# lucidrains/vit-pytorch

Hardware: NVIDIA H100
Metric: images/sec ViT-B/16 224^2 bf16 fwd (higher is better)
Workload: dtype bf16

## Files before the change

vit_pytorch_b200/csrc/attention.cu:

```cuda
#include "common.cuh"
#include "host_util.h"

namespace b200 {

constexpr int ATT_QROWS = 128;
constexpr int ATT_THREADS = 256;

struct AttnParams {
  __nv_bfloat16* out;
  int N;
  const int32_t* cu_seqlens;
  const int32_t* tile_prefix;
  int num_seqs;
  int H, I;
  float scale_log2e;
};

template <int DH, int KB>
struct AttnSmem {
  static constexpr int N64 = DH / 64;
  static constexpr int N16 = (DH % 64) / 16;
  static_assert(N64 * 64 + N16 * 16 == DH, "dim_head must be a multiple of 16");
  static constexpr int Q64 = ATT_QROWS * 128;
  static constexpr int Q16 = ATT_QROWS * 32;
  static constexpr int KV64 = KB * 128;
  static constexpr int KV16 = KB * 32;
  static constexpr int K16_OFF = 2 * N64 * KV64;
  static constexpr int V16_OFF = K16_OFF + N16 * KV16;
  static constexpr int STAGE = 2 * (N64 * KV64 + N16 * KV16);
  static constexpr int STAGE_OFF = N64 * Q64 + N16 * Q16;
  static constexpr int BAR_OFF = STAGE_OFF + 2 * STAGE;
  static constexpr int BYTES = BAR_OFF + 5 * 8 + 1024;
};

constexpr int att_min_blocks(int dh, int kb) { return (dh == 64 && kb == 64) || dh == 32 ? 2 : 1; }

template <int DH, int KB, bool VARLEN, bool EMUL, bool MASK_SELF>
__global__ void __launch_bounds__(ATT_THREADS, att_min_blocks(DH, KB))
attention_kernel(const __grid_constant__ CUtensorMap tmQ, const __grid_constant__ CUtensorMap tmKV,
                 const __grid_constant__ CUtensorMap tmQ16, const __grid_constant__ CUtensorMap tmKV16,
                 const AttnParams p) {
  using L = AttnSmem<DH, KB>;
  constexpr int N64 = L::N64, N16 = L::N16;
  constexpr int NS = KB / 2;
  extern __shared__ uint8_t smem_raw[];
  uint8_t* smem = reinterpret_cast<uint8_t*>((reinterpret_cast<uintptr_t>(smem_raw) + 1023) & ~uintptr_t(1023));
  uint64_t* full = reinterpret_cast<uint64_t*>(smem + L::BAR_OFF);
  uint64_t* empty = full + 2;
  uint64_t* qbar = full + 4;

  const int h = blockIdx.y;
  int seq_start, len, q0;
  if (VARLEN) {
    const int tile = blockIdx.x;
    int lo = 0, hi = p.num_seqs - 1;
    while (lo < hi) {
      const int mid = (lo + hi + 1) >> 1;
      if (p.tile_prefix[mid] <= tile) lo = mid;
      else hi = mid - 1;
    }
    seq_start = p.cu_seqlens[lo];
    len = p.cu_seqlens[lo + 1] - seq_start;
    q0 = (tile - p.tile_prefix[lo]) * ATT_QROWS;
  } else {
    seq_start = blockIdx.z * p.N;
    len = p.N;
    q0 = blockIdx.x * ATT_QROWS;
  }
  const int nblocks = (len + KB - 1) / KB;
  const int colq = h * DH, colk = p.I + h * DH, colv = 2 * p.I + h * DH;
  const int tid = threadIdx.x;
  const int wg = tid >> 7, t = tid & 127, warp = t >> 5, lane = t & 31;

  auto issue_kv = [&](int blk) {
    const int st = blk & 1;
    uint8_t* sb = smem + L::STAGE_OFF + st * L::STAGE;
    const int row = seq_start + blk * KB;
    mbar_arrive_expect_tx(&full[st], L::STAGE);
#pragma unroll
    for (int c = 0; c < N64; ++c) {
      tma_load_2d(sb + c * L::KV64, &tmKV, &full[st], colk + 64 * c, row);
      tma_load_2d(sb + (N64 + c) * L::KV64, &tmKV, &full[st], colv + 64 * c, row);
    }
#pragma unroll
    for (int c = 0; c < N16; ++c) {
      tma_load_2d(sb + L::K16_OFF + c * L::KV16, &tmKV16, &full[st], colk + 64 * N64 + 16 * c, row);
      tma_load_2d(sb + L::V16_OFF + c * L::KV16, &tmKV16, &full[st], colv + 64 * N64 + 16 * c, row);
    }
  };

  if (tid == 0) {
    tma_prefetch_desc(&tmQ);
    tma_prefetch_desc(&tmKV);
    for (int i = 0; i < 2; ++i) {
      mbar_init(&full[i], 1);
      mbar_init(&empty[i], 2);
    }
    mbar_init(qbar, 1);
    fence_mbar_init();
  }
  __syncthreads();
  if (tid == 0) {
    mbar_arrive_expect_tx(qbar, L::STAGE_OFF);
#pragma unroll
    for (int c = 0; c < N64; ++c) tma_load_2d(smem + c * L::Q64, &tmQ, qbar, colq + 64 * c, seq_start + q0);
#pragma unroll
    for (int c = 0; c < N16; ++c)
      tma_load_2d(smem + N64 * L::Q64 + c * L::Q16, &tmQ16, qbar, colq + 64 * N64 + 16 * c, seq_start + q0);
    issue_kv(0);
    if (nblocks > 1) issue_kv(1);
  }

  float o[N64 > 0 ? N64 : 1][32], o16[N16 > 0 ? N16 : 1][8];
#pragma unroll
  for (int c = 0; c < N64; ++c)
#pragma unroll
    for (int i = 0; i < 32; ++i) o[c][i] = 0.f;
#pragma unroll
  for (int c = 0; c < N16; ++c)
#pragma unroll
    for (int i = 0; i < 8; ++i) o16[c][i] = 0.f;
  float m[2] = {-INFINITY, -INFINITY}, l[2] = {0.f, 0.f};
  const uint32_t qa = smem_u32(smem) + wg * 64 * 128;
  const uint32_t qa16 = smem_u32(smem + N64 * L::Q64) + wg * 64 * 32;
  const bool mask_self = MASK_SELF && len > 1;
  mbar_wait(qbar, 0);

  for (int kb = 0; kb < nblocks; ++kb) {
    const int st = kb & 1;
    const uint32_t ph = (kb >> 1) & 1;
    mbar_wait(&full[st], ph);
    const uint32_t sb = smem_u32(smem + L::STAGE_OFF + st * L::STAGE);

    float s[NS];
    wgmma_fence();
#pragma unroll
    for (int c = 0; c < N64; ++c)
#pragma unroll
      for (int k = 0; k < 4; ++k) {
        const uint64_t ad = make_wgmma_desc(qa + c * L::Q64, 1024, WGMMA_SW128) + 2 * k;
        const uint64_t bd = make_wgmma_desc(sb + c * L::KV64, 1024, WGMMA_SW128) + 2 * k;
        if constexpr (KB == 128) wgmma_m64n128k16(s, ad, bd, c != 0 || k != 0);
        else wgmma_m64n64k16(s, ad, bd, c != 0 || k != 0);
      }
#pragma unroll
    for (int c = 0; c < N16; ++c) {
      const uint64_t ad = make_wgmma_desc(qa16 + c * L::Q16, 256, WGMMA_SW32);
      const uint64_t bd = make_wgmma_desc(sb + L::K16_OFF + c * L::KV16, 256, WGMMA_SW32);
      if constexpr (KB == 128) wgmma_m64n128k16(s, ad, bd, N64 != 0 || c != 0);
      else wgmma_m64n64k16(s, ad, bd, N64 != 0 || c != 0);
    }
    wgmma_commit();
    wgmma_wait<0>();
    fence_regs(s);

    const int key0 = kb * KB + 2 * (lane & 3);
    float mx[2] = {m[0], m[1]};
#pragma unroll
    for (int j = 0; j < KB / 8; ++j)
#pragma unroll
      for (int e = 0; e < 4; ++e) {
        const int key = key0 + j * 8 + (e & 1);
        bool valid = key < len;
        if constexpr (MASK_SELF)
          valid = valid && !(mask_self && key == q0 + wg * 64 + warp * 16 + (lane >> 2) + 8 * (e >> 1));
        s[4 * j + e] = valid ? s[4 * j + e] * p.scale_log2e : -INFINITY;
        mx[e >> 1] = fmaxf(mx[e >> 1], s[4 * j + e]);
      }
#pragma unroll
    for (int r = 0; r < 2; ++r) {
      mx[r] = fmaxf(mx[r], __shfl_xor_sync(0xffffffffu, mx[r], 1));
      mx[r] = fmaxf(mx[r], __shfl_xor_sync(0xffffffffu, mx[r], 2));
      const float corr = fast_ex2(m[r] - mx[r]);
      l[r] *= corr;
#pragma unroll
      for (int c = 0; c < N64; ++c)
#pragma unroll
        for (int i = 0; i < 8; ++i) {
          o[c][4 * i + 2 * r] *= corr;
          o[c][4 * i + 2 * r + 1] *= corr;
        }
#pragma unroll
      for (int c = 0; c < N16; ++c)
#pragma unroll
        for (int i = 0; i < 2; ++i) {
          o16[c][4 * i + 2 * r] *= corr;
          o16[c][4 * i + 2 * r + 1] *= corr;
        }
      m[r] = mx[r];
    }
#pragma unroll
    for (int j = 0; j < KB / 8; ++j) {
#pragma unroll
      for (int r = 0; r < 2; ++r) {
        float e0, e1;
        const float x0 = s[4 * j + 2 * r] - m[r], x1 = s[4 * j + 2 * r + 1] - m[r];
        if (EMUL && (j & 1)) {
          exp2_emul2(f2_make(x0, x1), e0, e1);
          e0 = s[4 * j + 2 * r] == -INFINITY ? 0.f : e0;
          e1 = s[4 * j + 2 * r + 1] == -INFINITY ? 0.f : e1;
        } else {
          e0 = fast_ex2(x0);
          e1 = fast_ex2(x1);
        }
        s[4 * j + 2 * r] = e0;
        s[4 * j + 2 * r + 1] = e1;
        l[r] += e0 + e1;
      }
    }

    wgmma_fence();
#pragma unroll
    for (int kk = 0; kk < KB / 16; ++kk) {
      const uint32_t a[4] = {pack_bf16x2(s[8 * kk], s[8 * kk + 1]), pack_bf16x2(s[8 * kk + 2], s[8 * kk + 3]),
                             pack_bf16x2(s[8 * kk + 4], s[8 * kk + 5]), pack_bf16x2(s[8 * kk + 6], s[8 * kk + 7])};
#pragma unroll
      for (int c = 0; c < N64; ++c)
        wgmma_m64n64k16_rs_tb(o[c], a,
                              make_wgmma_desc_lbo(sb + (N64 + c) * L::KV64 + kk * 2048, 1024, 1024, WGMMA_SW128));
#pragma unroll
      for (int c = 0; c < N16; ++c)
        wgmma_m64n16k16_rs_tb(o16[c], a,
                              make_wgmma_desc_lbo(sb + L::V16_OFF + c * L::KV16 + kk * 512, 256, 256, WGMMA_SW32));
    }
    wgmma_commit();
    wgmma_wait<0>();
#pragma unroll
    for (int c = 0; c < N64; ++c) fence_regs(o[c]);
#pragma unroll
    for (int c = 0; c < N16; ++c) fence_regs(o16[c]);
    if (t == 0) mbar_arrive(&empty[st]);
    if (tid == 0 && kb + 2 < nblocks) {
      mbar_wait(&empty[st], ph);
      issue_kv(kb + 2);
    }
  }

#pragma unroll
  for (int r = 0; r < 2; ++r) {
    l[r] += __shfl_xor_sync(0xffffffffu, l[r], 1);
    l[r] += __shfl_xor_sync(0xffffffffu, l[r], 2);
    l[r] = 1.0f / l[r];
  }
  const int qr = q0 + wg * 64 + warp * 16 + (lane >> 2);
#pragma unroll
  for (int r = 0; r < 2; ++r) {
    const int row = qr + 8 * r;
    if (row >= len) continue;
    __nv_bfloat16* op = p.out + (long long)(seq_start + row) * p.I + h * DH + 2 * (lane & 3);
#pragma unroll
    for (int c = 0; c < N64; ++c)
#pragma unroll
      for (int j = 0; j < 8; ++j)
        *reinterpret_cast<uint32_t*>(op + 64 * c + j * 8) =
            pack_bf16x2(o[c][4 * j + 2 * r] * l[r], o[c][4 * j + 2 * r + 1] * l[r]);
#pragma unroll
    for (int c = 0; c < N16; ++c)
#pragma unroll
      for (int j = 0; j < 2; ++j)
        *reinterpret_cast<uint32_t*>(op + 64 * N64 + 16 * c + j * 8) =
            pack_bf16x2(o16[c][4 * j + 2 * r] * l[r], o16[c][4 * j + 2 * r + 1] * l[r]);
  }
}

template <int DH, int KB, bool VARLEN, bool EMUL, bool MASK_SELF>
static int launch_attention_t(const void* qkv, int T, const AttnParams& p, dim3 grid, cudaStream_t stream) {
  using L = AttnSmem<DH, KB>;
  CUtensorMap tm[4];
  const uint64_t dims[2] = {(uint64_t)3 * p.I, (uint64_t)T};
  const uint64_t strides[1] = {(uint64_t)3 * p.I * 2};
  const uint32_t qbox[2] = {64, ATT_QROWS}, kvbox[2] = {64, KB}, qbox16[2] = {16, ATT_QROWS}, kvbox16[2] = {16, KB};
  int rc = 0;
  if (L::N64) rc = encode_tmap_bf16(&tm[0], qkv, 2, dims, strides, qbox);
  if (!rc && L::N64) rc = encode_tmap_bf16(&tm[1], qkv, 2, dims, strides, kvbox);
  if (!rc && L::N16) rc = encode_tmap_bf16_sw(&tm[2], qkv, 2, dims, strides, qbox16, 32);
  if (!rc && L::N16) rc = encode_tmap_bf16_sw(&tm[3], qkv, 2, dims, strides, kvbox16, 32);
  if (rc) return rc;
  if (!L::N16) tm[2] = tm[0], tm[3] = tm[1];
  if (!L::N64) tm[0] = tm[2], tm[1] = tm[3];
  auto kern = attention_kernel<DH, KB, VARLEN, EMUL, MASK_SELF>;
  B200_ENSURE_SMEM(kern, L::BYTES);
  kern<<<grid, ATT_THREADS, L::BYTES, stream>>>(tm[0], tm[1], tm[2], tm[3], p);
  B200_CHECK_CUDA(cudaGetLastError());
  count_launch();
  return 0;
}

template <int DH, bool VARLEN>
static int launch_attention_dh(const void* qkv, int T, const AttnParams& p, int kb, bool emul, bool mask_self,
                               dim3 grid, cudaStream_t st) {
  if (mask_self) return launch_attention_t<DH, 64, VARLEN, false, true>(qkv, T, p, grid, st);
  if (kb == 128) return emul ? launch_attention_t<DH, 128, VARLEN, true, false>(qkv, T, p, grid, st)
                             : launch_attention_t<DH, 128, VARLEN, false, false>(qkv, T, p, grid, st);
  return emul ? launch_attention_t<DH, 64, VARLEN, true, false>(qkv, T, p, grid, st)
              : launch_attention_t<DH, 64, VARLEN, false, false>(qkv, T, p, grid, st);
}

template <bool VARLEN>
static int launch_attention(const void* qkv, int T, const AttnParams& p, int dh, int kb, bool emul, bool mask_self,
                            dim3 grid, cudaStream_t st) {
  switch (dh) {
    case 32: return launch_attention_dh<32, VARLEN>(qkv, T, p, kb, emul, mask_self, grid, st);
    case 80: return launch_attention_dh<80, VARLEN>(qkv, T, p, kb, emul, mask_self, grid, st);
    case 128: return launch_attention_dh<128, VARLEN>(qkv, T, p, kb, emul, mask_self, grid, st);
    default: return launch_attention_dh<64, VARLEN>(qkv, T, p, kb, emul, mask_self, grid, st);
  }
}

static std::atomic<int> g_attn_mode{0};
static std::atomic<int> g_attn_emul{0};
static std::atomic<int> g_varlen_mode{0};

}

using namespace b200;

extern "C" int b200vit_debug_set(int key, int value) {
  switch (key) {
    case 1: g_attn_mode = value; return 0;
    case 11: g_varlen_mode = value; return 0;
    case 12: gemm_set_block_n(value); return 0;
    case 13: g_attn_emul = value; return 0;
    case 14: gemm_set_direct_store(value); return 0;
    default: return B200VIT_ERR_INVALID;
  }
}

extern "C" int b200vit_attention(const void* qkv, void* out, int B, int N, int H, int dh, float scale, void* stream) {
  return b200vit_attention_ex(qkv, out, B, N, H, dh, scale, 0, stream);
}

extern "C" int b200vit_attention_ex(const void* qkv, void* out, int B, int N, int H, int dh, float scale, int flags,
                                    void* stream) {
  B200_CHECK_ARG(qkv && out, "attention: null pointer");
  B200_CHECK_ARG(B > 0 && N > 0 && H > 0, "attention: bad shape B=%d N=%d H=%d", B, N, H);
  B200_CHECK_ARG(head_width_ok(dh), "attention: dim_head=%d not supported by this build (32, 64, 80 or 128)", dh);
  B200_CHECK_ARG(N <= 512, "attention: N=%d > 512 goes through b200vit_attention_varlen", N);
  B200_CHECK_ARG((reinterpret_cast<uintptr_t>(qkv) & 15) == 0 && (reinterpret_cast<uintptr_t>(out) & 15) == 0,
                 "attention: pointers must be 16-byte aligned");
  B200_CHECK_ARG(B <= 65535, "attention: B=%d exceeds the grid", B);
  B200_CHECK_ARG((flags & ~B200VIT_ATTN_MASK_SELF) == 0, "attention: unknown flags 0x%x", flags);
  AttnParams p{};
  p.out = reinterpret_cast<__nv_bfloat16*>(out);
  p.N = N;
  p.H = H;
  p.I = H * dh;
  p.scale_log2e = scale * 1.4426950408889634f;
  const dim3 grid((N + ATT_QROWS - 1) / ATT_QROWS, H, B);
  return launch_attention<false>(qkv, B * N, p, dh, g_attn_mode.load() == 2 ? 128 : 64, g_attn_emul.load() != 0,
                                 (flags & B200VIT_ATTN_MASK_SELF) != 0, grid, reinterpret_cast<cudaStream_t>(stream));
}

extern "C" int b200vit_attention_varlen(const void* qkv, void* out, const int32_t* cu_seqlens_dev,
                                        const int32_t* tile_prefix_dev, int num_seqs, int total_tokens, int total_tiles,
                                        int H, int dh, float scale, void* stream) {
  return b200vit_attention_varlen_ex(qkv, out, cu_seqlens_dev, tile_prefix_dev, num_seqs, total_tokens, total_tiles, H,
                                     dh, scale, 0, stream);
}

extern "C" int b200vit_attention_varlen_ex(const void* qkv, void* out, const int32_t* cu_seqlens_dev,
                                           const int32_t* tile_prefix_dev, int num_seqs, int total_tokens,
                                           int total_tiles, int H, int dh, float scale, int flags, void* stream) {
  B200_CHECK_ARG(qkv && out && cu_seqlens_dev && tile_prefix_dev, "attention_varlen: null pointer");
  B200_CHECK_ARG(num_seqs > 0 && total_tokens > 0 && total_tiles > 0 && H > 0, "attention_varlen: bad shape");
  B200_CHECK_ARG(head_width_ok(dh), "attention_varlen: dim_head=%d not supported by this build (32, 64, 80 or 128)",
                 dh);
  B200_CHECK_ARG((reinterpret_cast<uintptr_t>(qkv) & 15) == 0 && (reinterpret_cast<uintptr_t>(out) & 15) == 0,
                 "attention_varlen: pointers must be 16-byte aligned");
  B200_CHECK_ARG(H <= 65535, "attention_varlen: H=%d exceeds the grid", H);
  B200_CHECK_ARG((flags & ~B200VIT_ATTN_MASK_SELF) == 0, "attention_varlen: unknown flags 0x%x", flags);
  AttnParams p{};
  p.out = reinterpret_cast<__nv_bfloat16*>(out);
  p.cu_seqlens = cu_seqlens_dev;
  p.tile_prefix = tile_prefix_dev;
  p.num_seqs = num_seqs;
  p.H = H;
  p.I = H * dh;
  p.scale_log2e = scale * 1.4426950408889634f;
  const int mode = g_varlen_mode.load();
  const dim3 grid(total_tiles, H, 1);
  return launch_attention<true>(qkv, total_tokens, p, dh, mode == 1 ? 128 : 64, mode == 2,
                                (flags & B200VIT_ATTN_MASK_SELF) != 0, grid, reinterpret_cast<cudaStream_t>(stream));
}
```

vit_pytorch_b200/csrc/common.cuh:

```cuda
#pragma once
#include <cuda.h>
#include <cuda_runtime.h>
#include <cuda_bf16.h>
#include <stdint.h>

namespace b200 {

__device__ __forceinline__ uint32_t smem_u32(const void* p) {
  return static_cast<uint32_t>(__cvta_generic_to_shared(p));
}
__device__ __forceinline__ uint64_t globaltimer_ns() {
  uint64_t t;
  asm volatile("mov.u64 %0, %%globaltimer;" : "=l"(t));
  return t;
}
__device__ __forceinline__ bool elect_one() {
  uint32_t pred;
  asm volatile(
      "{\n\t.reg .pred p;\n\t"
      "elect.sync _|p, 0xffffffff;\n\t"
      "selp.u32 %0, 1, 0, p;\n\t}"
      : "=r"(pred));
  return pred != 0;
}

__device__ __forceinline__ void pdl_wait() { asm volatile("griddepcontrol.wait;" ::: "memory"); }
__device__ __forceinline__ void pdl_launch_dependents() { asm volatile("griddepcontrol.launch_dependents;" ::: "memory"); }

template <int N>
__device__ __forceinline__ void setmaxnreg_inc() { asm volatile("setmaxnreg.inc.sync.aligned.u32 %0;" ::"n"(N)); }
template <int N>
__device__ __forceinline__ void setmaxnreg_dec() { asm volatile("setmaxnreg.dec.sync.aligned.u32 %0;" ::"n"(N)); }

__device__ __forceinline__ void mbar_init(uint64_t* bar, uint32_t count) {
  asm volatile("mbarrier.init.shared::cta.b64 [%0], %1;" ::"r"(smem_u32(bar)), "r"(count) : "memory");
}
__device__ __forceinline__ void fence_mbar_init() {
  asm volatile("fence.mbarrier_init.release.cluster;" ::: "memory");
}
__device__ __forceinline__ void sts_v4(uint32_t addr, uint32_t x, uint32_t y, uint32_t z, uint32_t w) {
  asm volatile("st.shared.v4.b32 [%0], {%1, %2, %3, %4};" ::"r"(addr), "r"(x), "r"(y), "r"(z), "r"(w) : "memory");
}
__device__ __forceinline__ void sts_v4f(uint32_t addr, float x, float y, float z, float w) {
  asm volatile("st.shared.v4.f32 [%0], {%1, %2, %3, %4};" ::"r"(addr), "f"(x), "f"(y), "f"(z), "f"(w) : "memory");
}
__device__ __forceinline__ float4 lds_v4f(uint32_t addr) {
  float4 r;
  asm volatile("ld.shared.v4.f32 {%0, %1, %2, %3}, [%4];" : "=f"(r.x), "=f"(r.y), "=f"(r.z), "=f"(r.w) : "r"(addr) : "memory");
  return r;
}
__device__ __forceinline__ void fence_proxy_async_smem() {
  asm volatile("fence.proxy.async.shared::cta;" ::: "memory");
}
__device__ __forceinline__ void mbar_arrive_expect_tx(uint64_t* bar, uint32_t bytes) {
  asm volatile("mbarrier.arrive.expect_tx.shared::cta.b64 _, [%0], %1;" ::"r"(smem_u32(bar)), "r"(bytes) : "memory");
}
__device__ __forceinline__ void mbar_arrive(uint64_t* bar) {
  asm volatile("mbarrier.arrive.shared::cta.b64 _, [%0];" ::"r"(smem_u32(bar)) : "memory");
}
__device__ __forceinline__ uint32_t mbar_try_wait(uint64_t* bar, uint32_t parity) {
  uint32_t ok;
  asm volatile(
      "{\n\t.reg .pred p;\n\t"
      "mbarrier.try_wait.parity.shared::cta.b64 p, [%1], %2;\n\t"
      "selp.u32 %0, 1, 0, p;\n\t}"
      : "=r"(ok)
      : "r"(smem_u32(bar)), "r"(parity)
      : "memory");
  return ok;
}
#ifndef B200VIT_WATCHDOG_NS
#define B200VIT_WATCHDOG_NS 4000000000ull
#endif
__device__ __forceinline__ void mbar_wait(uint64_t* bar, uint32_t parity) {
  if (mbar_try_wait(bar, parity)) return;
  uint64_t t0 = globaltimer_ns();
  uint32_t spins = 0;
  while (!mbar_try_wait(bar, parity)) {
    if (((++spins) & 0x3FFu) == 0) {
      if (globaltimer_ns() - t0 > B200VIT_WATCHDOG_NS) __trap();
    }
  }
}

__device__ __forceinline__ void tma_prefetch_desc(const CUtensorMap* tm) {
  asm volatile("prefetch.tensormap [%0];" ::"l"(reinterpret_cast<uint64_t>(tm)) : "memory");
}
__device__ __forceinline__ void tma_prefetch_l2_2d(const CUtensorMap* tm, int c0, int c1) {
  asm volatile("cp.async.bulk.prefetch.tensor.2d.L2.global.tile [%0, {%1, %2}];" ::"l"(reinterpret_cast<uint64_t>(tm)),
               "r"(c0), "r"(c1)
               : "memory");
}
__device__ __forceinline__ void tma_load_2d(void* smem_dst, const CUtensorMap* tm, uint64_t* bar, int c0, int c1) {
  asm volatile(
      "cp.async.bulk.tensor.2d.shared::cluster.global.mbarrier::complete_tx::bytes [%0], [%1, {%3, %4}], [%2];"
      ::"r"(smem_u32(smem_dst)), "l"(reinterpret_cast<uint64_t>(tm)), "r"(smem_u32(bar)), "r"(c0), "r"(c1)
      : "memory");
}
__device__ __forceinline__ void tma_load_3d(void* smem_dst, const CUtensorMap* tm, uint64_t* bar, int c0, int c1,
                                            int c2) {
  asm volatile(
      "cp.async.bulk.tensor.3d.shared::cluster.global.mbarrier::complete_tx::bytes [%0], [%1, {%3, %4, %5}], [%2];"
      ::"r"(smem_u32(smem_dst)), "l"(reinterpret_cast<uint64_t>(tm)), "r"(smem_u32(bar)), "r"(c0), "r"(c1), "r"(c2)
      : "memory");
}
__device__ __forceinline__ void tma_load_4d(void* smem_dst, const CUtensorMap* tm, uint64_t* bar, int c0, int c1,
                                            int c2, int c3) {
  asm volatile(
      "cp.async.bulk.tensor.4d.shared::cluster.global.mbarrier::complete_tx::bytes [%0], [%1, {%3, %4, %5, %6}], [%2];"
      ::"r"(smem_u32(smem_dst)), "l"(reinterpret_cast<uint64_t>(tm)), "r"(smem_u32(bar)), "r"(c0), "r"(c1), "r"(c2),
      "r"(c3)
      : "memory");
}
__device__ __forceinline__ void tma_load_5d(void* smem_dst, const CUtensorMap* tm, uint64_t* bar, int c0, int c1,
                                            int c2, int c3, int c4) {
  asm volatile(
      "cp.async.bulk.tensor.5d.shared::cluster.global.mbarrier::complete_tx::bytes [%0], [%1, {%3, %4, %5, %6, %7}], "
      "[%2];"
      ::"r"(smem_u32(smem_dst)), "l"(reinterpret_cast<uint64_t>(tm)), "r"(smem_u32(bar)), "r"(c0), "r"(c1), "r"(c2),
      "r"(c3), "r"(c4)
      : "memory");
}
__device__ __forceinline__ void tma_store_2d(const CUtensorMap* tm, const void* smem_src, int c0, int c1) {
  asm volatile("cp.async.bulk.tensor.2d.global.shared::cta.bulk_group [%0, {%2, %3}], [%1];" ::"l"(
                   reinterpret_cast<uint64_t>(tm)),
               "r"(smem_u32(smem_src)), "r"(c0), "r"(c1)
               : "memory");
}
__device__ __forceinline__ void tma_store_commit() { asm volatile("cp.async.bulk.commit_group;" ::: "memory"); }
template <int N>
__device__ __forceinline__ void tma_store_wait_read() {
  asm volatile("cp.async.bulk.wait_group.read %0;" ::"n"(N) : "memory");
}
template <int N>
__device__ __forceinline__ void tma_store_wait() {
  asm volatile("cp.async.bulk.wait_group %0;" ::"n"(N) : "memory");
}

__device__ __forceinline__ uint64_t make_wgmma_desc(uint32_t smem_addr, uint32_t sbo_bytes, uint32_t swizzle) {
  uint64_t d = 0;
  d |= static_cast<uint64_t>((smem_addr & 0x3FFFFu) >> 4);
  d |= static_cast<uint64_t>(1u) << 16;
  d |= static_cast<uint64_t>((sbo_bytes >> 4) & 0x3FFFu) << 32;
  d |= static_cast<uint64_t>(swizzle) << 62;
  return d;
}
__device__ __forceinline__ uint64_t make_wgmma_desc_lbo(uint32_t smem_addr, uint32_t lbo_bytes, uint32_t sbo_bytes,
                                                        uint32_t swizzle) {
  return (make_wgmma_desc(smem_addr, sbo_bytes, swizzle) & ~(0x3FFFull << 16)) |
         (static_cast<uint64_t>((lbo_bytes >> 4) & 0x3FFFu) << 16);
}
constexpr uint32_t WGMMA_SW128 = 1;
constexpr uint32_t WGMMA_SW32 = 3;

__device__ __forceinline__ void wgmma_fence() { asm volatile("wgmma.fence.sync.aligned;" ::: "memory"); }
__device__ __forceinline__ void wgmma_commit() { asm volatile("wgmma.commit_group.sync.aligned;" ::: "memory"); }
template <int N>
__device__ __forceinline__ void wgmma_wait() { asm volatile("wgmma.wait_group.sync.aligned %0;" ::"n"(N) : "memory"); }
template <int R>
__device__ __forceinline__ void fence_regs(float (&d)[R]) {
#pragma unroll
  for (int i = 0; i < R; ++i) asm volatile("" : "+f"(d[i])::"memory");
}

__device__ __forceinline__ void wgmma_m64n128k16(float (&d)[64], uint64_t a_desc, uint64_t b_desc, uint32_t scale_d) {
  asm volatile(
      "{\n\t.reg .pred p;\n\t"
      "setp.ne.b32 p, %66, 0;\n\t"
      "wgmma.mma_async.sync.aligned.m64n128k16.f32.bf16.bf16 "
      "{"
      "%0, %1, %2, %3, %4, %5, %6, %7, %8, %9, %10, %11, %12, %13, %14, %15, "
      "%16, %17, %18, %19, %20, %21, %22, %23, %24, %25, %26, %27, %28, %29, %30, %31, "
      "%32, %33, %34, %35, %36, %37, %38, %39, %40, %41, %42, %43, %44, %45, %46, %47, "
      "%48, %49, %50, %51, %52, %53, %54, %55, %56, %57, %58, %59, %60, %61, %62, %63"
      "}, %64, %65, p, 1, 1, 0, 0;\n\t}"
      : "+f"(d[0]), "+f"(d[1]), "+f"(d[2]), "+f"(d[3]), "+f"(d[4]), "+f"(d[5]), "+f"(d[6]), "+f"(d[7]),
        "+f"(d[8]), "+f"(d[9]), "+f"(d[10]), "+f"(d[11]), "+f"(d[12]), "+f"(d[13]), "+f"(d[14]), "+f"(d[15]),
        "+f"(d[16]), "+f"(d[17]), "+f"(d[18]), "+f"(d[19]), "+f"(d[20]), "+f"(d[21]), "+f"(d[22]), "+f"(d[23]),
        "+f"(d[24]), "+f"(d[25]), "+f"(d[26]), "+f"(d[27]), "+f"(d[28]), "+f"(d[29]), "+f"(d[30]), "+f"(d[31]),
        "+f"(d[32]), "+f"(d[33]), "+f"(d[34]), "+f"(d[35]), "+f"(d[36]), "+f"(d[37]), "+f"(d[38]), "+f"(d[39]),
        "+f"(d[40]), "+f"(d[41]), "+f"(d[42]), "+f"(d[43]), "+f"(d[44]), "+f"(d[45]), "+f"(d[46]), "+f"(d[47]),
        "+f"(d[48]), "+f"(d[49]), "+f"(d[50]), "+f"(d[51]), "+f"(d[52]), "+f"(d[53]), "+f"(d[54]), "+f"(d[55]),
        "+f"(d[56]), "+f"(d[57]), "+f"(d[58]), "+f"(d[59]), "+f"(d[60]), "+f"(d[61]), "+f"(d[62]), "+f"(d[63])
      : "l"(a_desc), "l"(b_desc), "r"(scale_d));
}
__device__ __forceinline__ void wgmma_m64n256k16(float (&d)[128], uint64_t a_desc, uint64_t b_desc, uint32_t scale_d) {
  asm volatile(
      "{\n\t.reg .pred p;\n\t"
      "setp.ne.b32 p, %130, 0;\n\t"
      "wgmma.mma_async.sync.aligned.m64n256k16.f32.bf16.bf16 "
      "{"
      "%0, %1, %2, %3, %4, %5, %6, %7, %8, %9, %10, %11, %12, %13, %14, %15, "
      "%16, %17, %18, %19, %20, %21, %22, %23, %24, %25, %26, %27, %28, %29, %30, %31, "
      "%32, %33, %34, %35, %36, %37, %38, %39, %40, %41, %42, %43, %44, %45, %46, %47, "
      "%48, %49, %50, %51, %52, %53, %54, %55, %56, %57, %58, %59, %60, %61, %62, %63, "
      "%64, %65, %66, %67, %68, %69, %70, %71, %72, %73, %74, %75, %76, %77, %78, %79, "
      "%80, %81, %82, %83, %84, %85, %86, %87, %88, %89, %90, %91, %92, %93, %94, %95, "
      "%96, %97, %98, %99, %100, %101, %102, %103, %104, %105, %106, %107, %108, %109, %110, %111, "
      "%112, %113, %114, %115, %116, %117, %118, %119, %120, %121, %122, %123, %124, %125, %126, %127"
      "}, %128, %129, p, 1, 1, 0, 0;\n\t}"
      : "+f"(d[0]), "+f"(d[1]), "+f"(d[2]), "+f"(d[3]), "+f"(d[4]), "+f"(d[5]), "+f"(d[6]), "+f"(d[7]),
        "+f"(d[8]), "+f"(d[9]), "+f"(d[10]), "+f"(d[11]), "+f"(d[12]), "+f"(d[13]), "+f"(d[14]), "+f"(d[15]),
        "+f"(d[16]), "+f"(d[17]), "+f"(d[18]), "+f"(d[19]), "+f"(d[20]), "+f"(d[21]), "+f"(d[22]), "+f"(d[23]),
        "+f"(d[24]), "+f"(d[25]), "+f"(d[26]), "+f"(d[27]), "+f"(d[28]), "+f"(d[29]), "+f"(d[30]), "+f"(d[31]),
        "+f"(d[32]), "+f"(d[33]), "+f"(d[34]), "+f"(d[35]), "+f"(d[36]), "+f"(d[37]), "+f"(d[38]), "+f"(d[39]),
        "+f"(d[40]), "+f"(d[41]), "+f"(d[42]), "+f"(d[43]), "+f"(d[44]), "+f"(d[45]), "+f"(d[46]), "+f"(d[47]),
        "+f"(d[48]), "+f"(d[49]), "+f"(d[50]), "+f"(d[51]), "+f"(d[52]), "+f"(d[53]), "+f"(d[54]), "+f"(d[55]),
        "+f"(d[56]), "+f"(d[57]), "+f"(d[58]), "+f"(d[59]), "+f"(d[60]), "+f"(d[61]), "+f"(d[62]), "+f"(d[63]),
        "+f"(d[64]), "+f"(d[65]), "+f"(d[66]), "+f"(d[67]), "+f"(d[68]), "+f"(d[69]), "+f"(d[70]), "+f"(d[71]),
        "+f"(d[72]), "+f"(d[73]), "+f"(d[74]), "+f"(d[75]), "+f"(d[76]), "+f"(d[77]), "+f"(d[78]), "+f"(d[79]),
        "+f"(d[80]), "+f"(d[81]), "+f"(d[82]), "+f"(d[83]), "+f"(d[84]), "+f"(d[85]), "+f"(d[86]), "+f"(d[87]),
        "+f"(d[88]), "+f"(d[89]), "+f"(d[90]), "+f"(d[91]), "+f"(d[92]), "+f"(d[93]), "+f"(d[94]), "+f"(d[95]),
        "+f"(d[96]), "+f"(d[97]), "+f"(d[98]), "+f"(d[99]), "+f"(d[100]), "+f"(d[101]), "+f"(d[102]), "+f"(d[103]),
        "+f"(d[104]), "+f"(d[105]), "+f"(d[106]), "+f"(d[107]), "+f"(d[108]), "+f"(d[109]), "+f"(d[110]), "+f"(d[111]),
        "+f"(d[112]), "+f"(d[113]), "+f"(d[114]), "+f"(d[115]), "+f"(d[116]), "+f"(d[117]), "+f"(d[118]), "+f"(d[119]),
        "+f"(d[120]), "+f"(d[121]), "+f"(d[122]), "+f"(d[123]), "+f"(d[124]), "+f"(d[125]), "+f"(d[126]), "+f"(d[127])
      : "l"(a_desc), "l"(b_desc), "r"(scale_d));
}


__device__ __forceinline__ void wgmma_m64n64k16(float (&d)[32], uint64_t a_desc, uint64_t b_desc, uint32_t scale_d) {
  asm volatile(
      "{\n\t.reg .pred p;\n\t"
      "setp.ne.b32 p, %34, 0;\n\t"
      "wgmma.mma_async.sync.aligned.m64n64k16.f32.bf16.bf16 "
      "{"
      "%0, %1, %2, %3, %4, %5, %6, %7, %8, %9, %10, %11, %12, %13, %14, %15, "
      "%16, %17, %18, %19, %20, %21, %22, %23, %24, %25, %26, %27, %28, %29, %30, %31"
      "}, %32, %33, p, 1, 1, 0, 0;\n\t}"
      : "+f"(d[0]), "+f"(d[1]), "+f"(d[2]), "+f"(d[3]), "+f"(d[4]), "+f"(d[5]), "+f"(d[6]), "+f"(d[7]),
        "+f"(d[8]), "+f"(d[9]), "+f"(d[10]), "+f"(d[11]), "+f"(d[12]), "+f"(d[13]), "+f"(d[14]), "+f"(d[15]),
        "+f"(d[16]), "+f"(d[17]), "+f"(d[18]), "+f"(d[19]), "+f"(d[20]), "+f"(d[21]), "+f"(d[22]), "+f"(d[23]),
        "+f"(d[24]), "+f"(d[25]), "+f"(d[26]), "+f"(d[27]), "+f"(d[28]), "+f"(d[29]), "+f"(d[30]), "+f"(d[31])
      : "l"(a_desc), "l"(b_desc), "r"(scale_d));
}
__device__ __forceinline__ void wgmma_m64n64k16_rs_tb(float (&d)[32], const uint32_t (&a)[4], uint64_t b_desc) {
  asm volatile(
      "{\n\t.reg .pred p;\n\t"
      "setp.ne.b32 p, 1, 0;\n\t"
      "wgmma.mma_async.sync.aligned.m64n64k16.f32.bf16.bf16 "
      "{"
      "%0, %1, %2, %3, %4, %5, %6, %7, %8, %9, %10, %11, %12, %13, %14, %15, "
      "%16, %17, %18, %19, %20, %21, %22, %23, %24, %25, %26, %27, %28, %29, %30, %31"
      "}, {%32, %33, %34, %35}, %36, p, 1, 1, 1;\n\t}"
      : "+f"(d[0]), "+f"(d[1]), "+f"(d[2]), "+f"(d[3]), "+f"(d[4]), "+f"(d[5]), "+f"(d[6]), "+f"(d[7]),
        "+f"(d[8]), "+f"(d[9]), "+f"(d[10]), "+f"(d[11]), "+f"(d[12]), "+f"(d[13]), "+f"(d[14]), "+f"(d[15]),
        "+f"(d[16]), "+f"(d[17]), "+f"(d[18]), "+f"(d[19]), "+f"(d[20]), "+f"(d[21]), "+f"(d[22]), "+f"(d[23]),
        "+f"(d[24]), "+f"(d[25]), "+f"(d[26]), "+f"(d[27]), "+f"(d[28]), "+f"(d[29]), "+f"(d[30]), "+f"(d[31])
      : "r"(a[0]), "r"(a[1]), "r"(a[2]), "r"(a[3]), "l"(b_desc));
}
__device__ __forceinline__ void wgmma_m64n16k16_rs_tb(float (&d)[8], const uint32_t (&a)[4], uint64_t b_desc) {
  asm volatile(
      "{\n\t.reg .pred p;\n\t"
      "setp.ne.b32 p, 1, 0;\n\t"
      "wgmma.mma_async.sync.aligned.m64n16k16.f32.bf16.bf16 "
      "{"
      "%0, %1, %2, %3, %4, %5, %6, %7"
      "}, {%8, %9, %10, %11}, %12, p, 1, 1, 1;\n\t}"
      : "+f"(d[0]), "+f"(d[1]), "+f"(d[2]), "+f"(d[3]), "+f"(d[4]), "+f"(d[5]), "+f"(d[6]), "+f"(d[7])
      : "r"(a[0]), "r"(a[1]), "r"(a[2]), "r"(a[3]), "l"(b_desc));
}



__device__ __forceinline__ float fast_rcp(float x) {
  float r;
  asm("rcp.approx.ftz.f32 %0, %1;" : "=f"(r) : "f"(x));
  return r;
}
__device__ __forceinline__ float fast_ex2(float x) {
  float r;
  asm("ex2.approx.ftz.f32 %0, %1;" : "=f"(r) : "f"(x));
  return r;
}

__device__ __forceinline__ uint32_t pack_bf16x2(float lo, float hi) {
  __nv_bfloat162 v = __floats2bfloat162_rn(lo, hi);
  return *reinterpret_cast<uint32_t*>(&v);
}
typedef float2 f32x2;
__device__ __forceinline__ f32x2 f2_make(float a, float b) { return make_float2(a, b); }
__device__ __forceinline__ void f2_get(f32x2 v, float& a, float& b) {
  a = v.x;
  b = v.y;
}
__device__ __forceinline__ f32x2 f2_fma(f32x2 a, f32x2 b, f32x2 c) {
  return make_float2(__fmaf_rn(a.x, b.x, c.x), __fmaf_rn(a.y, b.y, c.y));
}
__device__ __forceinline__ f32x2 f2_mul(f32x2 a, f32x2 b) { return make_float2(__fmul_rn(a.x, b.x), __fmul_rn(a.y, b.y)); }
__device__ __forceinline__ f32x2 f2_add(f32x2 a, f32x2 b) { return make_float2(__fadd_rn(a.x, b.x), __fadd_rn(a.y, b.y)); }

__device__ __forceinline__ void exp2_emul2(f32x2 x, float& e0, float& e1) {
  float x0, x1;
  f2_get(x, x0, x1);
  x = f2_make(fmaxf(x0, -125.0f), fmaxf(x1, -125.0f));
  const f32x2 t = f2_add(x, f2_make(12582912.0f, 12582912.0f));
  const f32x2 n = f2_add(t, f2_make(-12582912.0f, -12582912.0f));
  const f32x2 f = f2_fma(n, f2_make(-1.0f, -1.0f), x);
  f32x2 pl = f2_fma(f2_make(0.05517210811376572f, 0.05517210811376572f), f,
                    f2_make(0.24261118471622467f, 0.24261118471622467f));
  pl = f2_fma(pl, f, f2_make(0.693260908126831f, 0.693260908126831f));
  pl = f2_fma(pl, f, f2_make(0.9999280571937561f, 0.9999280571937561f));
  float p0, p1, t0, t1;
  f2_get(pl, p0, p1);
  f2_get(t, t0, t1);
  e0 = __uint_as_float(__float_as_uint(p0) + (__float_as_uint(t0) << 23));
  e1 = __uint_as_float(__float_as_uint(p1) + (__float_as_uint(t1) << 23));
}

__device__ __forceinline__ float gelu_erf(float x) {
  const float x2 = fminf(x * x, 36.0f);
  float p = 2.4836384909576736e-05f;
  p = fmaf(p, x2, 7.3606101796031e-04f);
  p = fmaf(p, x2, -1.0598272830247879e-01f);
  p = fmaf(p, x2, -2.301647186279297f);
  const float e = fast_ex2(p * x);
  return x * fast_rcp(1.0f + e);
}
__device__ __forceinline__ void gelu_erf2(float& a, float& b) {
  const f32x2 x = f2_make(a, b);
  float t0, t1;
  f2_get(f2_mul(x, x), t0, t1);
  const f32x2 x2 = f2_make(fminf(t0, 36.0f), fminf(t1, 36.0f));
  f32x2 p = f2_fma(f2_make(2.4836384909576736e-05f, 2.4836384909576736e-05f), x2,
                   f2_make(7.3606101796031e-04f, 7.3606101796031e-04f));
  p = f2_fma(p, x2, f2_make(-1.0598272830247879e-01f, -1.0598272830247879e-01f));
  p = f2_fma(p, x2, f2_make(-2.301647186279297f, -2.301647186279297f));
  float u0, u1;
  f2_get(f2_mul(p, x), u0, u1);
  const f32x2 d = f2_add(f2_make(fast_ex2(u0), fast_ex2(u1)), f2_make(1.0f, 1.0f));
  float d0, d1;
  f2_get(d, d0, d1);
  f2_get(f2_mul(x, f2_make(fast_rcp(d0), fast_rcp(d1))), a, b);
}

}
```

vit_pytorch_b200/csrc/host_util.h:

```cpp
#pragma once
#include <cuda.h>
#include <cuda_runtime.h>
#include <stdint.h>
#include <atomic>
#include <cstdarg>
#include <cstdio>
#include <utility>

#include "../../include/b200vit.h"

namespace b200 {

void set_error(const char* fmt, ...);
extern std::atomic<int64_t> g_launches;
inline void count_launch(int n = 1) { g_launches.fetch_add(n, std::memory_order_relaxed); }

#define B200_CHECK_ARG(cond, ...)        \
  do {                                   \
    if (!(cond)) {                       \
      b200::set_error(__VA_ARGS__);      \
      return B200VIT_ERR_INVALID;        \
    }                                    \
  } while (0)

#define B200_CHECK_CUDA(expr)                                                                     \
  do {                                                                                            \
    cudaError_t _e = (expr);                                                                      \
    if (_e != cudaSuccess) {                                                                      \
      b200::set_error("%s failed: %s (%s:%d)", #expr, cudaGetErrorString(_e), __FILE__, __LINE__); \
      return B200VIT_ERR_CUDA;                                                                    \
    }                                                                                             \
  } while (0)

int encode_tmap_bf16(CUtensorMap* tm, const void* base, int rank, const uint64_t* dims, const uint64_t* strides_bytes,
                     const uint32_t* box, bool swizzle128 = true);
int encode_tmap_bf16_sw(CUtensorMap* tm, const void* base, int rank, const uint64_t* dims,
                        const uint64_t* strides_bytes, const uint32_t* box, int swizzle_bytes);
int encode_tmap_f32(CUtensorMap* tm, const void* base, int rank, const uint64_t* dims, const uint64_t* strides_bytes,
                    const uint32_t* box, bool swizzle128 = false);

void tmap_cache_stats(int64_t* hits, int64_t* misses);

inline bool head_width_ok(int dh) { return dh == 32 || dh == 64 || dh == 80 || dh == 128; }

void gemm_set_block_n(int v);
void gemm_set_direct_store(int v);

int num_sms();
bool pdl_enabled();
template <typename... KArgs, typename... Args>
inline cudaError_t launch_kernel(void (*kern)(KArgs...), dim3 grid, dim3 block, size_t smem, cudaStream_t stream,
                                 bool pdl, Args&&... args) {
  cudaLaunchConfig_t cfg{};
  cfg.gridDim = grid;
  cfg.blockDim = block;
  cfg.dynamicSmemBytes = smem;
  cfg.stream = stream;
  cudaLaunchAttribute attr[1];
  attr[0].id = cudaLaunchAttributeProgrammaticStreamSerialization;
  attr[0].val.programmaticStreamSerializationAllowed = 1;
  cfg.attrs = attr;
  cfg.numAttrs = (pdl && pdl_enabled()) ? 1 : 0;
  return cudaLaunchKernelEx(&cfg, kern, std::forward<Args>(args)...);
}
int ensure_dyn_smem(const void* kernel, size_t bytes);
#define B200_ENSURE_SMEM(kern, bytes)                                                       \
  do {                                                                                      \
    int _rc = b200::ensure_dyn_smem(reinterpret_cast<const void*>(kern), (size_t)(bytes));  \
    if (_rc) return _rc;                                                                    \
  } while (0)

}
```

Baseline: 8221.

## Add persistent one-pass attention kernel for short sequences with dim_head 64

Adds a specialized attention kernel for dh=64 and N<=256 that loads the whole Q, K and V for a (batch, head) unit into shared memory via TMA. It computes softmax in a single pass with no online rescaling across key blocks. A producer warpgroup double-buffers units while two consumer warpgroups process 64-row query strips with n208/n256 wgmma. This aims to remove the rescaling overhead and per-tile launch granularity of the general flash kernel, at the cost of high register and shared-memory use and one CTA per SM.

New measurement: 8458, median of 6. 1.03x the previous value.

```diff
diff --git a/vit_pytorch_b200/csrc/attention.cu b/vit_pytorch_b200/csrc/attention.cu
--- a/vit_pytorch_b200/csrc/attention.cu
+++ b/vit_pytorch_b200/csrc/attention.cu
@@ -310,6 +310,7 @@
 static std::atomic<int> g_attn_mode{0};
 static std::atomic<int> g_attn_emul{0};
 static std::atomic<int> g_varlen_mode{0};
+static std::atomic<int> g_attn_streaming{0};
 
 }
 
@@ -322,6 +323,7 @@
     case 12: gemm_set_block_n(value); return 0;
     case 13: g_attn_emul = value; return 0;
     case 14: gemm_set_direct_store(value); return 0;
+    case 15: g_attn_streaming = value; return 0;
     default: return B200VIT_ERR_INVALID;
   }
 }
@@ -346,9 +348,14 @@
   p.H = H;
   p.I = H * dh;
   p.scale_log2e = scale * 1.4426950408889634f;
+  const bool mask_self = (flags & B200VIT_ATTN_MASK_SELF) != 0;
+  const int mode = g_attn_mode.load();
+  const bool emul = g_attn_emul.load() != 0;
+  if (dh == 64 && N <= 256 && scale > 0.f && !mask_self && mode == 0 && !emul && g_attn_streaming.load() == 0)
+    return launch_attention_onepass(qkv, out, B, N, H, p.scale_log2e, reinterpret_cast<cudaStream_t>(stream));
   const dim3 grid((N + ATT_QROWS - 1) / ATT_QROWS, H, B);
-  return launch_attention<false>(qkv, B * N, p, dh, g_attn_mode.load() == 2 ? 128 : 64, g_attn_emul.load() != 0,
-                                 (flags & B200VIT_ATTN_MASK_SELF) != 0, grid, reinterpret_cast<cudaStream_t>(stream));
+  return launch_attention<false>(qkv, B * N, p, dh, mode == 2 ? 128 : 64, emul, mask_self, grid,
+                                 reinterpret_cast<cudaStream_t>(stream));
 }
 
 extern "C" int b200vit_attention_varlen(const void* qkv, void* out, const int32_t* cu_seqlens_dev,
diff --git a/vit_pytorch_b200/csrc/attention_short.cu b/vit_pytorch_b200/csrc/attention_short.cu
--- /dev/null
+++ b/vit_pytorch_b200/csrc/attention_short.cu
@@ -0,0 +1,202 @@
+#include "common.cuh"
+#include "host_util.h"
+
+namespace b200 {
+
+constexpr int AO_THREADS = 384;
+
+template <int KT>
+struct OnepassSmem {
+  static constexpr int QROWS = (KT + 63) / 64 * 64;
+  static constexpr int K_OFF = QROWS * 128;
+  static constexpr int V_OFF = K_OFF + KT * 128;
+  static constexpr int UNIT = V_OFF + KT * 128;
+  static constexpr int BAR_OFF = 2 * UNIT;
+  static constexpr int BYTES = BAR_OFF + 4 * 8 + 1024;
+  static_assert(KT % 16 == 0 && KT <= 256, "key tile: a multiple of 16 up to 256");
+};
+
+struct OnepassParams {
+  __nv_bfloat16* out;
+  int N, H, I, units;
+  float scale_log2e;
+};
+
+template <int KT>
+__device__ __forceinline__ void wgmma_qk(float (&s)[KT / 2], uint64_t ad, uint64_t bd, uint32_t scale_d) {
+  if constexpr (KT == 256) wgmma_m64n256k16(s, ad, bd, scale_d);
+  else if constexpr (KT == 208) wgmma_m64n208k16(s, ad, bd, scale_d);
+  else if constexpr (KT == 128) wgmma_m64n128k16(s, ad, bd, scale_d);
+  else wgmma_m64n64k16(s, ad, bd, scale_d);
+}
+
+template <int KT>
+__global__ void __launch_bounds__(AO_THREADS, 1)
+attention_onepass_kernel(const __grid_constant__ CUtensorMap tmQ, const __grid_constant__ CUtensorMap tmKV,
+                         const OnepassParams p) {
+  using L = OnepassSmem<KT>;
+  constexpr int NS = KT / 2;
+  extern __shared__ uint8_t smem_raw[];
+  uint8_t* smem = smem_raw + ((1024u - (smem_u32(smem_raw) & 1023u)) & 1023u);
+  uint64_t* full = reinterpret_cast<uint64_t*>(smem + L::BAR_OFF);
+  uint64_t* empty = full + 2;
+  const int wg = threadIdx.x >> 7;
+
+  if (threadIdx.x == 0) {
+    tma_prefetch_desc(&tmQ);
+    tma_prefetch_desc(&tmKV);
+    for (int i = 0; i < 2; ++i) {
+      mbar_init(&full[i], 1);
+      mbar_init(&empty[i], 2);
+    }
+    fence_mbar_init();
+  }
+  __syncthreads();
+
+  if (wg == 0) {
+    setmaxnreg_dec<40>();
+    if (threadIdx.x == 0) {
+      int it = 0;
+      for (int u = blockIdx.x; u < p.units; u += gridDim.x, ++it) {
+        const int buf = it & 1;
+        mbar_wait(&empty[buf], ((it >> 1) & 1) ^ 1);
+        const int b = u / p.H, col = (u % p.H) * 64;
+        uint8_t* sb = smem + buf * L::UNIT;
+        mbar_arrive_expect_tx(&full[buf], L::UNIT);
+        tma_load_3d(sb, &tmQ, &full[buf], col, 0, b);
+        tma_load_3d(sb + L::K_OFF, &tmKV, &full[buf], p.I + col, 0, b);
+        tma_load_3d(sb + L::V_OFF, &tmKV, &full[buf], 2 * p.I + col, 0, b);
+      }
+    }
+    return;
+  }
+
+  setmaxnreg_inc<232>();
+  const int c = wg - 1;
+  const int t = threadIdx.x & 127, warp = t >> 5, lane = t & 31;
+  const int N = p.N;
+  const int nstrips = (N + 63) / 64;
+  int it = 0;
+  for (int u = blockIdx.x; u < p.units; u += gridDim.x, ++it) {
+    const int buf = it & 1;
+    const int b = u / p.H, h = u % p.H;
+    mbar_wait(&full[buf], (it >> 1) & 1);
+    if (c >= nstrips && t == 0) mbar_arrive(&empty[buf]);
+    const uint32_t sq = smem_u32(smem + buf * L::UNIT);
+    for (int s = c; s < nstrips; s += 2) {
+      float sc[NS];
+      wgmma_fence();
+#pragma unroll
+      for (int k = 0; k < 4; ++k)
+        wgmma_qk<KT>(sc, make_wgmma_desc(sq + s * 64 * 128, 1024, WGMMA_SW128) + 2 * k,
+                     make_wgmma_desc(sq + L::K_OFF, 1024, WGMMA_SW128) + 2 * k, k != 0);
+      wgmma_commit();
+      wgmma_wait<0>();
+      fence_regs(sc);
+
+      constexpr int KT_VALID = KT == 256 ? 208 : KT == 208 ? 128 : KT == 128 ? 64 : 0;
+      const int key0 = 2 * (lane & 3);
+      float mx[2] = {-INFINITY, -INFINITY};
+#pragma unroll
+      for (int j = 0; j < KT / 8; ++j)
+#pragma unroll
+        for (int e = 0; e < 4; ++e) {
+          if (8 * j + 8 > KT_VALID && key0 + 8 * j + (e & 1) >= N) sc[4 * j + e] = -INFINITY;
+          mx[e >> 1] = fmaxf(mx[e >> 1], sc[4 * j + e]);
+        }
+#pragma unroll
+      for (int r = 0; r < 2; ++r) {
+        mx[r] = fmaxf(mx[r], __shfl_xor_sync(0xffffffffu, mx[r], 1));
+        mx[r] = fmaxf(mx[r], __shfl_xor_sync(0xffffffffu, mx[r], 2));
+        mx[r] *= -p.scale_log2e;
+      }
+      float l[2] = {0.f, 0.f};
+      uint32_t pk[KT / 4];
+      auto softmax_blocks = [&](int j0, int j1) {
+#pragma unroll
+        for (int j = j0; j < j1; ++j)
+#pragma unroll
+          for (int r = 0; r < 2; ++r) {
+            const float e0 = fast_ex2(fmaf(sc[4 * j + 2 * r], p.scale_log2e, mx[r]));
+            const float e1 = fast_ex2(fmaf(sc[4 * j + 2 * r + 1], p.scale_log2e, mx[r]));
+            pk[2 * j + r] = pack_bf16x2(e0, e1);
+            l[r] += e0 + e1;
+          }
+      };
+      constexpr int KH = KT == 256 ? KT / 16 : (KT / 16 + 1) / 2;
+      auto pv_steps = [&](float (&o)[32], int k0, int k1) {
+        wgmma_fence();
+#pragma unroll
+        for (int kk = k0; kk < k1; ++kk) {
+          const uint32_t a[4] = {pk[4 * kk], pk[4 * kk + 1], pk[4 * kk + 2], pk[4 * kk + 3]};
+          wgmma_m64n64k16_rs_tb(o, a, make_wgmma_desc_lbo(sq + L::V_OFF + kk * 2048, 1024, 1024, WGMMA_SW128));
+        }
+        wgmma_commit();
+      };
+      float o[32];
+#pragma unroll
+      for (int i = 0; i < 32; ++i) o[i] = 0.f;
+      softmax_blocks(0, 2 * KH);
+      pv_steps(o, 0, KH);
+      if constexpr (KH < KT / 16) {
+        softmax_blocks(2 * KH, KT / 8);
+        pv_steps(o, KH, KT / 16);
+      }
+      wgmma_wait<0>();
+      fence_regs(o);
+      if (s + 2 >= nstrips && t == 0) mbar_arrive(&empty[buf]);
+
+#pragma unroll
+      for (int r = 0; r < 2; ++r) {
+        l[r] += __shfl_xor_sync(0xffffffffu, l[r], 1);
+        l[r] += __shfl_xor_sync(0xffffffffu, l[r], 2);
+        l[r] = 1.0f / l[r];
+      }
+      const int qr = s * 64 + warp * 16 + (lane >> 2);
+#pragma unroll
+      for (int r = 0; r < 2; ++r) {
+        const int row = qr + 8 * r;
+        if (row >= N) continue;
+        __nv_bfloat16* op = p.out + ((long long)b * N + row) * p.I + h * 64 + 2 * (lane & 3);
+#pragma unroll
+        for (int j = 0; j < 8; ++j)
+          *reinterpret_cast<uint32_t*>(op + j * 8) = pack_bf16x2(o[4 * j + 2 * r] * l[r], o[4 * j + 2 * r + 1] * l[r]);
+      }
+    }
+  }
+}
+
+template <int KT>
+static int launch_onepass_t(const void* qkv, int B, const OnepassParams& p, cudaStream_t stream) {
+  using L = OnepassSmem<KT>;
+  const uint64_t dims[3] = {(uint64_t)3 * p.I, (uint64_t)p.N, (uint64_t)B};
+  const uint64_t strides[2] = {(uint64_t)3 * p.I * 2, (uint64_t)p.N * 3 * p.I * 2};
+  const uint32_t qbox[3] = {64, L::QROWS, 1}, kvbox[3] = {64, KT, 1};
+  CUtensorMap tmQ, tmKV;
+  int rc = encode_tmap_bf16(&tmQ, qkv, 3, dims, strides, qbox);
+  if (!rc) rc = encode_tmap_bf16(&tmKV, qkv, 3, dims, strides, kvbox);
+  if (rc) return rc;
+  auto kern = attention_onepass_kernel<KT>;
+  B200_ENSURE_SMEM(kern, L::BYTES);
+  const int grid = p.units < num_sms() ? p.units : num_sms();
+  kern<<<grid, AO_THREADS, L::BYTES, stream>>>(tmQ, tmKV, p);
+  B200_CHECK_CUDA(cudaGetLastError());
+  count_launch();
+  return 0;
+}
+
+int launch_attention_onepass(const void* qkv, void* out, int B, int N, int H, float scale_log2e, cudaStream_t stream) {
+  OnepassParams p{};
+  p.out = reinterpret_cast<__nv_bfloat16*>(out);
+  p.N = N;
+  p.H = H;
+  p.I = H * 64;
+  p.units = B * H;
+  p.scale_log2e = scale_log2e;
+  if (N <= 64) return launch_onepass_t<64>(qkv, B, p, stream);
+  if (N <= 128) return launch_onepass_t<128>(qkv, B, p, stream);
+  if (N <= 208) return launch_onepass_t<208>(qkv, B, p, stream);
+  return launch_onepass_t<256>(qkv, B, p, stream);
+}
+
+}
diff --git a/vit_pytorch_b200/csrc/common.cuh b/vit_pytorch_b200/csrc/common.cuh
--- a/vit_pytorch_b200/csrc/common.cuh
+++ b/vit_pytorch_b200/csrc/common.cuh
@@ -215,6 +215,36 @@
         "+f"(d[104]), "+f"(d[105]), "+f"(d[106]), "+f"(d[107]), "+f"(d[108]), "+f"(d[109]), "+f"(d[110]), "+f"(d[111]),
         "+f"(d[112]), "+f"(d[113]), "+f"(d[114]), "+f"(d[115]), "+f"(d[116]), "+f"(d[117]), "+f"(d[118]), "+f"(d[119]),
         "+f"(d[120]), "+f"(d[121]), "+f"(d[122]), "+f"(d[123]), "+f"(d[124]), "+f"(d[125]), "+f"(d[126]), "+f"(d[127])
+      : "l"(a_desc), "l"(b_desc), "r"(scale_d));
+}
+
+__device__ __forceinline__ void wgmma_m64n208k16(float (&d)[104], uint64_t a_desc, uint64_t b_desc, uint32_t scale_d) {
+  asm volatile(
+      "{\n\t.reg .pred p;\n\t"
+      "setp.ne.b32 p, %106, 0;\n\t"
+      "wgmma.mma_async.sync.aligned.m64n208k16.f32.bf16.bf16 "
+      "{"
+      "%0, %1, %2, %3, %4, %5, %6, %7, %8, %9, %10, %11, %12, %13, %14, %15, "
+      "%16, %17, %18, %19, %20, %21, %22, %23, %24, %25, %26, %27, %28, %29, %30, %31, "
+      "%32, %33, %34, %35, %36, %37, %38, %39, %40, %41, %42, %43, %44, %45, %46, %47, "
+      "%48, %49, %50, %51, %52, %53, %54, %55, %56, %57, %58, %59, %60, %61, %62, %63, "
+      "%64, %65, %66, %67, %68, %69, %70, %71, %72, %73, %74, %75, %76, %77, %78, %79, "
+      "%80, %81, %82, %83, %84, %85, %86, %87, %88, %89, %90, %91, %92, %93, %94, %95, "
+      "%96, %97, %98, %99, %100, %101, %102, %103"
+      "}, %104, %105, p, 1, 1, 0, 0;\n\t}"
+      : "+f"(d[0]), "+f"(d[1]), "+f"(d[2]), "+f"(d[3]), "+f"(d[4]), "+f"(d[5]), "+f"(d[6]), "+f"(d[7]),
+        "+f"(d[8]), "+f"(d[9]), "+f"(d[10]), "+f"(d[11]), "+f"(d[12]), "+f"(d[13]), "+f"(d[14]), "+f"(d[15]),
+        "+f"(d[16]), "+f"(d[17]), "+f"(d[18]), "+f"(d[19]), "+f"(d[20]), "+f"(d[21]), "+f"(d[22]), "+f"(d[23]),
+        "+f"(d[24]), "+f"(d[25]), "+f"(d[26]), "+f"(d[27]), "+f"(d[28]), "+f"(d[29]), "+f"(d[30]), "+f"(d[31]),
+        "+f"(d[32]), "+f"(d[33]), "+f"(d[34]), "+f"(d[35]), "+f"(d[36]), "+f"(d[37]), "+f"(d[38]), "+f"(d[39]),
+        "+f"(d[40]), "+f"(d[41]), "+f"(d[42]), "+f"(d[43]), "+f"(d[44]), "+f"(d[45]), "+f"(d[46]), "+f"(d[47]),
+        "+f"(d[48]), "+f"(d[49]), "+f"(d[50]), "+f"(d[51]), "+f"(d[52]), "+f"(d[53]), "+f"(d[54]), "+f"(d[55]),
+        "+f"(d[56]), "+f"(d[57]), "+f"(d[58]), "+f"(d[59]), "+f"(d[60]), "+f"(d[61]), "+f"(d[62]), "+f"(d[63]),
+        "+f"(d[64]), "+f"(d[65]), "+f"(d[66]), "+f"(d[67]), "+f"(d[68]), "+f"(d[69]), "+f"(d[70]), "+f"(d[71]),
+        "+f"(d[72]), "+f"(d[73]), "+f"(d[74]), "+f"(d[75]), "+f"(d[76]), "+f"(d[77]), "+f"(d[78]), "+f"(d[79]),
+        "+f"(d[80]), "+f"(d[81]), "+f"(d[82]), "+f"(d[83]), "+f"(d[84]), "+f"(d[85]), "+f"(d[86]), "+f"(d[87]),
+        "+f"(d[88]), "+f"(d[89]), "+f"(d[90]), "+f"(d[91]), "+f"(d[92]), "+f"(d[93]), "+f"(d[94]), "+f"(d[95]),
+        "+f"(d[96]), "+f"(d[97]), "+f"(d[98]), "+f"(d[99]), "+f"(d[100]), "+f"(d[101]), "+f"(d[102]), "+f"(d[103])
       : "l"(a_desc), "l"(b_desc), "r"(scale_d));
 }
 
diff --git a/vit_pytorch_b200/csrc/host_util.h b/vit_pytorch_b200/csrc/host_util.h
--- a/vit_pytorch_b200/csrc/host_util.h
+++ b/vit_pytorch_b200/csrc/host_util.h
@@ -46,6 +46,8 @@
 void gemm_set_block_n(int v);
 void gemm_set_direct_store(int v);
 
+int launch_attention_onepass(const void* qkv, void* out, int B, int N, int H, float scale_log2e, cudaStream_t stream);
+
 int num_sms();
 bool pdl_enabled();
 template <typename... KArgs, typename... Args>
```
